# argmaxinc/WhisperKit

Hardware: NVIDIA H100
Metric: RTFx (audio-sec/s) whisper-large-v3 greedy (higher is better)
Workload: dtype bf16

## Files before the change

### whisperkit_b200/csrc/decoder_ops.cu

```cuda
#include <curand_kernel.h>
#include <math.h>

#include <stdlib.h>

#include "common.cuh"
#include <algorithm>
#include "kernels.h"

namespace wk {

static constexpr int kMaxCtx = 224;

__device__ __forceinline__ float block_sum(float v, float* scratch) {
    v = warp_sum(v);
    const int warp = threadIdx.x >> 5, lane = threadIdx.x & 31, nw = (blockDim.x + 31) >> 5;
    __syncthreads();
    if (lane == 0) scratch[warp] = v;
    __syncthreads();
    float r = (lane < nw) ? scratch[lane] : 0.f;
    r = warp_sum(r);
    return r;
}
__device__ __forceinline__ float block_max(float v, float* scratch) {
    v = warp_max(v);
    const int warp = threadIdx.x >> 5, lane = threadIdx.x & 31, nw = (blockDim.x + 31) >> 5;
    __syncthreads();
    if (lane == 0) scratch[warp] = v;
    __syncthreads();
    float r = (lane < nw) ? scratch[lane] : -INFINITY;
    r = warp_max(r);
    return r;
}

__global__ void decode_slots_init_kernel(DecodeState st, RowParams* __restrict__ rp_dev, const int32_t* __restrict__ slot_ids,
                                         const int32_t* __restrict__ prompts, const RowParams* __restrict__ rp_new, BeamState bs) {
    const int i = blockIdx.x, b = slot_ids[i];
    const RowParams R = rp_new[i];
    const int n_prompt = R.prompt_len;
    for (int t = threadIdx.x; t < kMaxCtx; t += blockDim.x) {
        st.tokens[b * kMaxCtx + t] = t < n_prompt ? prompts[i * kMaxCtx + t] : 0;
        st.logprobs[b * kMaxCtx + t] = 0.f;
        if (bs.beam > 1) bs.anc[b * kMaxCtx + t] = b;
    }
    if (threadIdx.x == 0) {
        rp_dev[b] = R;
        st.n_tokens[b] = n_prompt;
        st.next_token[b] = n_prompt > 0 ? prompts[i * kMaxCtx + n_prompt - 1] : 0;
        st.done[b] = 0;
        st.first_low[b] = 0;
        st.steps[b] = 0;
        st.input_ids[b] = 0;
        st.error[b] = 0;
        st.lang_token[b] = -1;
        st.lang_logprob[b] = 0.f;
        st.lang_state[b] = R.detect == 2 ? kLangLead : 0;
        st.no_speech[b] = __int_as_float(0x7fc00000);
        if (bs.beam > 1) {
            bs.sum_lp[b] = 0.f;
            if (b % bs.group == 0) bs.n_fin[b / bs.group] = 0;
        }
    }
}

wk_status decode_slots_init(DecodeState st, RowParams* rp_dev, const int32_t* slot_ids, const int32_t* prompts, const RowParams* rp_new,
                            int n, cudaStream_t stream, BeamState beam) {
    if (n < 1) return WK_OK;
    decode_slots_init_kernel<<<n, 64, 0, stream>>>(st, rp_dev, slot_ids, prompts, rp_new, beam);
    count_launch();
    cudaError_t e = cudaGetLastError();
    if (e != cudaSuccess) { set_error("decode_slots_init launch: %s", cudaGetErrorString(e)); return WK_ERR_CUDA; }
    return WK_OK;
}

template <typename T>
__global__ void __launch_bounds__(256)
decoder_embed_ln_kernel(const T* __restrict__ emb, const float* __restrict__ pos_emb, const float* __restrict__ gamma,
                        const float* __restrict__ beta, DecodeState st, int vocab, int ts_begin, float* __restrict__ x,
                        T* __restrict__ xn, int d, const int32_t* __restrict__ explicit_pos) {
    __shared__ float scratch[32];
    const int b = blockIdx.x, tid = threadIdx.x;
    pdl_launch_dependents();
    pdl_wait();
    int tok, pos;
    if (explicit_pos) {
        tok = st.input_ids[b];
        pos = explicit_pos[b];
    } else {
        if (st.done[b]) return;
        const int step = st.steps[b];
        const int prompt_len = st.rp[b].prompt_len;
        pos = step;
        tok = st.next_token[b];
        bool overwrite = false;
        const int lang_state = st.lang_state[b];
        if (lang_state == kLangLead) {
            tok = st.rp[b].lead_token;
        } else if (step < prompt_len) {
            const int cur = st.tokens[b * kMaxCtx + step];
            const bool is_ts = cur >= ts_begin, pred_ts = tok >= ts_begin;
            if (!(step == prompt_len - 1 && is_ts && pred_ts)) tok = cur;
            else overwrite = true;
        }
        __syncthreads();
        if (tid == 0) {
            if (overwrite) st.tokens[b * kMaxCtx + step] = tok;
            st.input_ids[b] = tok;
            if (lang_state == kLangLeadRan) st.lang_state[b] = 0;
        }
    }
    tok = min(max(tok, 0), vocab - 1);
    float v[8];
    float s = 0.f;
#pragma unroll
    for (int k = 0; k < 8; ++k) {
        const int i = tid + k * 256;
        v[k] = 0.f;
        if (i < d) {
            v[k] = T16<T>::to_f(emb[(long long)tok * d + i]) + pos_emb[(long long)pos * d + i];
            x[(long long)b * d + i] = v[k];
            s += v[k];
        }
    }
    const float mean = block_sum(s, scratch) / d;
    float q = 0.f;
#pragma unroll
    for (int k = 0; k < 8; ++k) {
        const int i = tid + k * 256;
        if (i < d) { const float a = v[k] - mean; q += a * a; }
    }
    const float rstd = rsqrtf(block_sum(q, scratch) / d + 1e-5f);
#pragma unroll
    for (int k = 0; k < 8; ++k) {
        const int i = tid + k * 256;
        if (i < d) xn[(long long)b * d + i] = T16<T>::from_f((v[k] - mean) * rstd * gamma[i] + beta[i]);
    }
}

wk_status decoder_embed_ln(const void* emb16, const float* pos, const float* gamma, const float* beta, DecodeState st, int vocab,
                           int ts_begin, float* x, void* xn, int B, int d, int dtype, const int32_t* explicit_pos, cudaStream_t stream) {
    if (d > 2048) { set_error("decoder_embed_ln: d_model %d > 2048", d); return WK_ERR_INVALID_ARGUMENT; }
    if (dtype == WK_DTYPE_F16)
        launch_k(decoder_embed_ln_kernel<__half>, dim3(B), dim3(256), 0, stream, 1, (const __half*)emb16, pos, gamma, beta, st, vocab, ts_begin, x, (__half*)xn, d, explicit_pos);
    else
        launch_k(decoder_embed_ln_kernel<__nv_bfloat16>, dim3(B), dim3(256), 0, stream, 1, (const __nv_bfloat16*)emb16, pos, gamma, beta, st, vocab, ts_begin, x, (__nv_bfloat16*)xn, d, explicit_pos);
    count_launch();
    cudaError_t e = cudaGetLastError();
    if (e != cudaSuccess) { set_error("decoder_embed_ln launch: %s", cudaGetErrorString(e)); return WK_ERR_CUDA; }
    return WK_OK;
}

static constexpr int kReduceThreads = 320;
static constexpr int kMaxSplits = 20;

template <typename T>
__global__ void __launch_bounds__(kReduceThreads)
decoder_reduce_resid_ln_kernel(const float* __restrict__ partial, int splits, int Bp, const float* __restrict__ bias,
                               const float* __restrict__ gamma, const float* __restrict__ beta, float* __restrict__ x,
                               T* __restrict__ xn, int d) {
    __shared__ float scratch[32];
    const int b = blockIdx.x, tid = threadIdx.x;
    const int d4 = d >> 2;
    pdl_launch_dependents();
    pdl_wait();
    float4 v[2];
    float s = 0.f;
#pragma unroll
    for (int k = 0; k < 2; ++k) {
        const int i4 = tid + k * kReduceThreads;
        v[k] = make_float4(0.f, 0.f, 0.f, 0.f);
        if (i4 < d4) {
            float4 p[kMaxSplits];
#pragma unroll
            for (int sp = 0; sp < kMaxSplits; ++sp)
                if (sp < splits) p[sp] = __ldcg(reinterpret_cast<const float4*>(partial + ((long long)sp * Bp + b) * d) + i4);
            float4 a = reinterpret_cast<const float4*>(x + (long long)b * d)[i4];
            if (bias) {
                const float4 bb = __ldg(reinterpret_cast<const float4*>(bias) + i4);
                a.x += bb.x; a.y += bb.y; a.z += bb.z; a.w += bb.w;
            }
#pragma unroll
            for (int sp = 0; sp < kMaxSplits; ++sp)
                if (sp < splits) { a.x += p[sp].x; a.y += p[sp].y; a.z += p[sp].z; a.w += p[sp].w; }
            v[k] = a;
            reinterpret_cast<float4*>(x + (long long)b * d)[i4] = a;
            s += a.x + a.y + a.z + a.w;
        }
    }
    const float mean = block_sum(s, scratch) / d;
    float q = 0.f;
#pragma unroll
    for (int k = 0; k < 2; ++k) {
        const int i4 = tid + k * kReduceThreads;
        if (i4 < d4) {
            const float a0 = v[k].x - mean, a1 = v[k].y - mean, a2 = v[k].z - mean, a3 = v[k].w - mean;
            q += a0 * a0 + a1 * a1 + a2 * a2 + a3 * a3;
        }
    }
    const float rstd = rsqrtf(block_sum(q, scratch) / d + 1e-5f);
#pragma unroll
    for (int k = 0; k < 2; ++k) {
        const int i4 = tid + k * kReduceThreads;
        if (i4 < d4) {
            const float4 g = __ldg(reinterpret_cast<const float4*>(gamma) + i4), bb = __ldg(reinterpret_cast<const float4*>(beta) + i4);
            uint2 pk;
            pk.x = T16<T>::pack2((v[k].x - mean) * rstd * g.x + bb.x, (v[k].y - mean) * rstd * g.y + bb.y);
            pk.y = T16<T>::pack2((v[k].z - mean) * rstd * g.z + bb.z, (v[k].w - mean) * rstd * g.w + bb.w);
            reinterpret_cast<uint2*>(xn + (long long)b * d)[i4] = pk;
        }
    }
}

wk_status decoder_reduce_resid_ln(const float* partial, int splits, int Bp, const float* bias, const float* gamma,
                                  const float* beta, float* x, void* xn, int B, int d, int dtype, cudaStream_t stream) {
    if (splits > kMaxSplits || d > 8 * kReduceThreads || (d & 3)) {
        set_error("decoder_reduce_resid_ln: unsupported splits %d / d %d", splits, d);
        return WK_ERR_INVALID_ARGUMENT;
    }
    if (dtype == WK_DTYPE_F16)
        launch_k(decoder_reduce_resid_ln_kernel<__half>, dim3(B), dim3(kReduceThreads), 0, stream, 32, partial, splits, Bp, bias, gamma, beta, x, (__half*)xn, d);
    else
        launch_k(decoder_reduce_resid_ln_kernel<__nv_bfloat16>, dim3(B), dim3(kReduceThreads), 0, stream, 32, partial, splits, Bp, bias, gamma, beta, x, (__nv_bfloat16*)xn, d);
    count_launch();
    cudaError_t e = cudaGetLastError();
    if (e != cudaSuccess) { set_error("decoder_reduce_resid_ln launch: %s", cudaGetErrorString(e)); return WK_ERR_CUDA; }
    return WK_OK;
}

template <typename T>
__global__ void __launch_bounds__(256)
decoder_reduce_bias_gelu_kernel(const float* __restrict__ partial, int splits, int Bp, const float* __restrict__ bias,
                                T* __restrict__ out, int B, int n) {
    pdl_launch_dependents();
    pdl_wait();
    const long long idx = ((long long)blockIdx.x * blockDim.x + threadIdx.x) * 4;
    if (idx >= (long long)B * n) return;
    const int b = (int)(idx / n), i = (int)(idx - (long long)b * n);
    float4 a = *reinterpret_cast<const float4*>(bias + i);
    float4 p[8];
#pragma unroll
    for (int sp = 0; sp < 8; ++sp)
        if (sp < splits) p[sp] = __ldcg(reinterpret_cast<const float4*>(partial + ((long long)sp * Bp + b) * n + i));
#pragma unroll
    for (int sp = 0; sp < 8; ++sp)
        if (sp < splits) { a.x += p[sp].x; a.y += p[sp].y; a.z += p[sp].z; a.w += p[sp].w; }
    for (int sp = 8; sp < splits; ++sp) {
        const float4 pp = __ldcg(reinterpret_cast<const float4*>(partial + ((long long)sp * Bp + b) * n + i));
        a.x += pp.x; a.y += pp.y; a.z += pp.z; a.w += pp.w;
    }
    uint2 pk;
    pk.x = T16<T>::pack2(gelu_erf(a.x), gelu_erf(a.y));
    pk.y = T16<T>::pack2(gelu_erf(a.z), gelu_erf(a.w));
    *reinterpret_cast<uint2*>(out + (long long)b * n + i) = pk;
}

wk_status decoder_reduce_bias_gelu(const float* partial, int splits, int Bp, const float* bias, void* out, int B, int n,
                                   int dtype, cudaStream_t stream) {
    const long long threads = (long long)B * n / 4;
    const unsigned grid = (unsigned)((threads + 255) / 256);
    if (dtype == WK_DTYPE_F16)
        launch_k(decoder_reduce_bias_gelu_kernel<__half>, dim3(grid), dim3(256), 0, stream, 32, partial, splits, Bp, bias, (__half*)out, B, n);
    else
        launch_k(decoder_reduce_bias_gelu_kernel<__nv_bfloat16>, dim3(grid), dim3(256), 0, stream, 32, partial, splits, Bp, bias, (__nv_bfloat16*)out, B, n);
    count_launch();
    cudaError_t e = cudaGetLastError();
    if (e != cudaSuccess) { set_error("decoder_reduce_bias_gelu launch: %s", cudaGetErrorString(e)); return WK_ERR_CUDA; }
    return WK_OK;
}

template <typename T, bool kAnc>
__global__ void __launch_bounds__(128)
decoder_self_attention_kernel(const float* __restrict__ partial, int splits, int Bp, const float* __restrict__ bq,
                              const float* __restrict__ bv, T* __restrict__ kcache, T* __restrict__ vcache,
                              const int32_t* __restrict__ pos_ptr, const int32_t* __restrict__ done,
                              T* __restrict__ out, int B, int H, int max_len, const int32_t* __restrict__ anc) {
    __shared__ float sq[64], skc[64], svc[64];
    __shared__ float sp[kMaxCtx];
    __shared__ float red[4][64];
    __shared__ float sstat[8];
    const int tid = threadIdx.x, warp = tid >> 5, lane = tid & 31;
    const int bh = blockIdx.x, b = bh / H, h = bh % H;
    pdl_launch_dependents();
    pdl_wait();
    if (done != nullptr && done[b]) return;
    const int dm = H * 64;
    const int pos = pos_ptr[b];
    const int32_t* arow = kAnc ? anc + (long long)b * max_len : nullptr;
    const long long own = (long long)bh * max_len;
    auto row_of = [&](int t) -> long long { return kAnc ? ((long long)arow[t] * H + h) * max_len + t : own + t; };
    if (warp == 0) {
        const int e = 2 * lane;
        float2 q = make_float2(bq[h * 64 + e], bq[h * 64 + e + 1]);
        float2 k = make_float2(0.f, 0.f);
        float2 v = make_float2(bv[h * 64 + e], bv[h * 64 + e + 1]);
        for (int s = 0; s < splits; ++s) {
            const float* pr = partial + ((long long)s * Bp + b) * (3LL * dm) + h * 64 + e;
            const float2 pq = *reinterpret_cast<const float2*>(pr);
            const float2 pk = *reinterpret_cast<const float2*>(pr + dm);
            const float2 pv = *reinterpret_cast<const float2*>(pr + 2 * dm);
            q.x += pq.x; q.y += pq.y; k.x += pk.x; k.y += pk.y; v.x += pv.x; v.y += pv.y;
        }
        const uint32_t k16 = T16<T>::pack2(k.x, k.y), v16 = T16<T>::pack2(v.x, v.y);
        *reinterpret_cast<uint32_t*>(kcache + (own + pos) * 64 + e) = k16;
        *reinterpret_cast<uint32_t*>(vcache + (own + pos) * 64 + e) = v16;
        const float2 kr = T16<T>::unpack2(k16), vr = T16<T>::unpack2(v16);
        sq[e] = q.x; sq[e + 1] = q.y;
        skc[e] = kr.x; skc[e + 1] = kr.y;
        svc[e] = vr.x; svc[e + 1] = vr.y;
        const float self = warp_sum(q.x * kr.x + q.y * kr.y);
        if (lane == 0) sp[pos] = self * 0.125f;
    }
    __syncthreads();
    const int sub = lane & 7, rsel = lane >> 3;
    float qv[8];
#pragma unroll
    for (int j = 0; j < 8; ++j) qv[j] = sq[sub * 8 + j];
    const T* kb = kcache + sub * 8;
#pragma unroll 4
    for (int t0 = warp * 4; t0 < pos; t0 += 16) {
        const int t = t0 + rsel;
        float acc = 0.f;
        if (t < pos) {
            const uint4 u = *reinterpret_cast<const uint4*>(kb + row_of(t) * 64);
            const float2 a0 = T16<T>::unpack2(u.x), a1 = T16<T>::unpack2(u.y), a2 = T16<T>::unpack2(u.z), a3 = T16<T>::unpack2(u.w);
            acc = qv[0] * a0.x + qv[1] * a0.y + qv[2] * a1.x + qv[3] * a1.y + qv[4] * a2.x + qv[5] * a2.y + qv[6] * a3.x + qv[7] * a3.y;
        }
        acc += __shfl_xor_sync(0xffffffffu, acc, 1);
        acc += __shfl_xor_sync(0xffffffffu, acc, 2);
        acc += __shfl_xor_sync(0xffffffffu, acc, 4);
        if (sub == 0 && t < pos) sp[t] = acc * 0.125f;
    }
    __syncthreads();
    float mx = -INFINITY;
    for (int t = tid; t <= pos; t += 128) mx = fmaxf(mx, sp[t]);
    mx = warp_max(mx);
    if (lane == 0) sstat[warp] = mx;
    __syncthreads();
    mx = fmaxf(fmaxf(sstat[0], sstat[1]), fmaxf(sstat[2], sstat[3]));
    float sm = 0.f;
    for (int t = tid; t <= pos; t += 128) {
        const float pr = __expf(sp[t] - mx);
        sp[t] = pr;
        sm += pr;
    }
    sm = warp_sum(sm);
    if (lane == 0) sstat[4 + warp] = sm;
    __syncthreads();
    const float inv = 1.f / (sstat[4] + sstat[5] + sstat[6] + sstat[7]);
    float o8[8];
#pragma unroll
    for (int j = 0; j < 8; ++j) o8[j] = 0.f;
    const T* vb = vcache + sub * 8;
#pragma unroll 4
    for (int t0 = warp * 4; t0 < pos; t0 += 16) {
        const int t = t0 + rsel;
        if (t < pos) {
            const float pr = sp[t];
            const uint4 u = *reinterpret_cast<const uint4*>(vb + row_of(t) * 64);
            const float2 a0 = T16<T>::unpack2(u.x), a1 = T16<T>::unpack2(u.y), a2 = T16<T>::unpack2(u.z), a3 = T16<T>::unpack2(u.w);
            o8[0] += pr * a0.x; o8[1] += pr * a0.y; o8[2] += pr * a1.x; o8[3] += pr * a1.y;
            o8[4] += pr * a2.x; o8[5] += pr * a2.y; o8[6] += pr * a3.x; o8[7] += pr * a3.y;
        }
    }
#pragma unroll
    for (int j = 0; j < 8; ++j) {
        o8[j] += __shfl_xor_sync(0xffffffffu, o8[j], 8);
        o8[j] += __shfl_xor_sync(0xffffffffu, o8[j], 16);
    }
    if (rsel == 0) {
#pragma unroll
        for (int j = 0; j < 8; ++j) red[warp][sub * 8 + j] = o8[j];
    }
    __syncthreads();
    if (tid < 64) {
        const float o = red[0][tid] + red[1][tid] + red[2][tid] + red[3][tid] + sp[pos] * svc[tid];
        out[(long long)b * dm + h * 64 + tid] = T16<T>::from_f(o * inv);
    }
}

wk_status decoder_self_attention(const float* partial, int splits, int Bp, const float* bq, const float* bv, void* kcache,
                                 void* vcache, const int32_t* pos, const int32_t* done, void* out, int B, int H,
                                 int max_len, int dtype, cudaStream_t stream, const int32_t* anc) {
    if (max_len > kMaxCtx) { set_error("decoder_self_attention: max_len %d > %d", max_len, kMaxCtx); return WK_ERR_INVALID_ARGUMENT; }
    const unsigned grid = (unsigned)(B * H);
    if (dtype == WK_DTYPE_F16) {
        if (anc) launch_k(decoder_self_attention_kernel<__half, true>, dim3(grid), dim3(128), 0, stream, 2, partial, splits, Bp, bq, bv, (__half*)kcache, (__half*)vcache, pos, done, (__half*)out, B, H, max_len, anc);
        else launch_k(decoder_self_attention_kernel<__half, false>, dim3(grid), dim3(128), 0, stream, 2, partial, splits, Bp, bq, bv, (__half*)kcache, (__half*)vcache, pos, done, (__half*)out, B, H, max_len, anc);
    } else {
        if (anc) launch_k(decoder_self_attention_kernel<__nv_bfloat16, true>, dim3(grid), dim3(128), 0, stream, 2, partial, splits, Bp, bq, bv, (__nv_bfloat16*)kcache, (__nv_bfloat16*)vcache, pos, done, (__nv_bfloat16*)out, B, H, max_len, anc);
        else launch_k(decoder_self_attention_kernel<__nv_bfloat16, false>, dim3(grid), dim3(128), 0, stream, 2, partial, splits, Bp, bq, bv, (__nv_bfloat16*)kcache, (__nv_bfloat16*)vcache, pos, done, (__nv_bfloat16*)out, B, H, max_len, anc);
    }
    count_launch();
    cudaError_t e = cudaGetLastError();
    if (e != cudaSuccess) { set_error("decoder_self_attention launch: %s", cudaGetErrorString(e)); return WK_ERR_CUDA; }
    return WK_OK;
}

template <bool FP8> struct CrossCfg {
    static constexpr int kRowBytes = FP8 ? 64 : 128;
    static constexpr int kRows = FP8 ? 250 : 125;
    static constexpr int kStageBytes = kRows * kRowBytes;
    static constexpr int kStages = 2;
    static constexpr int kLanesPerRow = kRowBytes / 16;
    static constexpr int kRowsPerWarp = 32 / kLanesPerRow;
    static constexpr int kDims = 64 / kLanesPerRow;
};
static constexpr int kCrossRows = CrossCfg<false>::kRows;
static constexpr int kCrossThreads = 160;

__device__ __forceinline__ void fp8x16_to_f32(const uint4 u, float (&x)[16]) {
    const uint32_t w[4] = {u.x, u.y, u.z, u.w};
#pragma unroll
    for (int k = 0; k < 4; ++k) {
        uint32_t lo, hi;
        fp8x4_to_half2(w[k], lo, hi);
        const float2 a = T16<__half>::unpack2(lo), b = T16<__half>::unpack2(hi);
        x[4 * k] = a.x; x[4 * k + 1] = a.y; x[4 * k + 2] = b.x; x[4 * k + 3] = b.y;
    }
}
template <typename T, bool FP8>
__device__ __forceinline__ float cross_row_dot(const uint8_t* piece, const float (&qv)[CrossCfg<FP8>::kDims]) {
    const uint4 u = *reinterpret_cast<const uint4*>(piece);
    if constexpr (FP8) {
        float x[16];
        fp8x16_to_f32(u, x);
        float acc = 0.f;
#pragma unroll
        for (int j = 0; j < 16; ++j) acc = fmaf(qv[j], x[j], acc);
        return acc;
    } else {
        const float2 a0 = T16<T>::unpack2(u.x), a1 = T16<T>::unpack2(u.y), a2 = T16<T>::unpack2(u.z), a3 = T16<T>::unpack2(u.w);
        return qv[0] * a0.x + qv[1] * a0.y + qv[2] * a1.x + qv[3] * a1.y + qv[4] * a2.x + qv[5] * a2.y + qv[6] * a3.x + qv[7] * a3.y;
    }
}
template <typename T, bool FP8>
__device__ __forceinline__ void cross_row_axpy(const uint8_t* piece, float p, float (&acc)[CrossCfg<FP8>::kDims]) {
    const uint4 u = *reinterpret_cast<const uint4*>(piece);
    if constexpr (FP8) {
        float x[16];
        fp8x16_to_f32(u, x);
#pragma unroll
        for (int j = 0; j < 16; ++j) acc[j] = fmaf(p, x[j], acc[j]);
    } else {
        const float2 a0 = T16<T>::unpack2(u.x), a1 = T16<T>::unpack2(u.y), a2 = T16<T>::unpack2(u.z), a3 = T16<T>::unpack2(u.w);
        acc[0] += p * a0.x; acc[1] += p * a0.y; acc[2] += p * a1.x; acc[3] += p * a1.y;
        acc[4] += p * a2.x; acc[5] += p * a2.y; acc[6] += p * a3.x; acc[7] += p * a3.y;
    }
}

template <typename T, bool FP8>
__global__ void __launch_bounds__(kCrossThreads)
decoder_cross_attention_kernel(const float* __restrict__ partial, int splits, int Bp, const float* __restrict__ bq,
                               const uint8_t* __restrict__ kcross, const uint8_t* __restrict__ vcross, const float* __restrict__ kscale,
                               const float* __restrict__ vscale, T* __restrict__ out, int B, int H, int Tlen, const int32_t* __restrict__ done,
                               float* __restrict__ align_scratch, uint32_t align_mask, int kv_div) {
    using C = CrossCfg<FP8>;
    extern __shared__ __align__(128) uint8_t smem[];
    const int Tp = (Tlen + 3) & ~3;
    uint8_t* ring = smem;
    float* scores = reinterpret_cast<float*>(smem + C::kStages * C::kStageBytes);
    float* ksc = scores + Tp;
    float* vsc = ksc + Tp;
    float* sq = FP8 ? vsc + Tp : scores + Tp;
    float* red = sq + 64;
    uint64_t* full_bar = reinterpret_cast<uint64_t*>(red + 4 * 64 + 32);
    uint64_t* empty_bar = full_bar + C::kStages;
    uint64_t* scale_bar = empty_bar + C::kStages;

    const int tid = threadIdx.x, warp = tid >> 5, lane = tid & 31;
    const int beam_j = blockIdx.x % kv_div, wh = blockIdx.x / kv_div;
    const int win = wh / H, h = wh % H, b = win * kv_div + beam_j;
    const int kvh = win * H + h;
    const int dm = H * 64;
    const int chunks = Tlen / C::kRows;
    pdl_launch_dependents();
    const int ended = done != nullptr ? done[b] : 0;
    if (tid == 0) {
        for (int i = 0; i < C::kStages; ++i) { mbar_init(&full_bar[i], 1); mbar_init(&empty_bar[i], 4); }
        if constexpr (FP8) mbar_init(scale_bar, 1);
        fence_barrier_init();
    }
    __syncthreads();
    if (ended) { pdl_wait(); return; }

    if (warp == 4) {
        if (lane == 0) {
            if constexpr (FP8) {
                mbar_expect_tx(scale_bar, 2u * Tlen * 4);
                bulk_load_1d(ksc, kscale + (long long)kvh * Tlen, Tlen * 4, scale_bar);
                bulk_load_1d(vsc, vscale + (long long)kvh * Tlen, Tlen * 4, scale_bar);
            }
            const uint8_t* kb = kcross + (long long)kvh * Tlen * C::kRowBytes;
            const uint8_t* vb = vcross + (long long)kvh * Tlen * C::kRowBytes;
            for (int c = 0; c < 2 * chunks; ++c) {
                const int stage = c % C::kStages;
                const uint32_t ph = (c / C::kStages) & 1;
                mbar_wait(&empty_bar[stage], ph ^ 1);
                mbar_expect_tx(&full_bar[stage], C::kStageBytes);
                const uint8_t* src = c < chunks ? kb + (long long)c * C::kStageBytes : vb + (long long)(c - chunks) * C::kStageBytes;
                bulk_load_1d(ring + stage * C::kStageBytes, src, C::kStageBytes, &full_bar[stage]);
            }
        }
        return;
    }
    pdl_wait();
    if (tid < 64) {
        float q = bq[h * 64 + tid];
        for (int s = 0; s < splits; ++s) q += partial[((long long)s * Bp + b) * dm + h * 64 + tid];
        sq[tid] = q * 0.125f;
    }
    asm volatile("bar.sync 1, 128;" ::: "memory");
    const int sub = lane % C::kLanesPerRow;
    const int rsel = lane / C::kLanesPerRow;
    float qv[C::kDims];
#pragma unroll
    for (int j = 0; j < C::kDims; ++j) qv[j] = sq[sub * C::kDims + j];
    if constexpr (FP8) mbar_wait(scale_bar, 0);

    for (int c = 0; c < chunks; ++c) {
        const int stage = c % C::kStages;
        const uint32_t ph = (c / C::kStages) & 1;
        mbar_wait(&full_bar[stage], ph);
        const uint8_t* tile = ring + stage * C::kStageBytes;
#pragma unroll
        for (int i = 0; i < 8; ++i) {
            const int r = warp * C::kRowsPerWarp + rsel + 4 * C::kRowsPerWarp * i;
            float acc = 0.f;
            if (r < C::kRows) acc = cross_row_dot<T, FP8>(tile + r * C::kRowBytes + sub * 16, qv);
#pragma unroll
            for (int o = 1; o < C::kLanesPerRow; o <<= 1) acc += __shfl_xor_sync(0xffffffffu, acc, o);
            if (sub == 0 && r < C::kRows) scores[c * C::kRows + r] = FP8 ? acc * ksc[c * C::kRows + r] : acc;
        }
        __syncwarp();
        if (lane == 0) mbar_arrive(&empty_bar[stage]);
    }
    asm volatile("bar.sync 1, 128;" ::: "memory");
    float mx = -INFINITY;
    for (int t = tid; t < Tlen; t += 128) mx = fmaxf(mx, scores[t]);
    mx = warp_max(mx);
    if (lane == 0) red[warp] = mx;
    asm volatile("bar.sync 1, 128;" ::: "memory");
    mx = fmaxf(fmaxf(red[0], red[1]), fmaxf(red[2], red[3]));
    float sm = 0.f;
    for (int t = tid; t < Tlen; t += 128) {
        const float p = __expf(scores[t] - mx);
        scores[t] = p;
        sm += p;
    }
    sm = warp_sum(sm);
    asm volatile("bar.sync 1, 128;" ::: "memory");
    if (lane == 0) red[warp] = sm;
    asm volatile("bar.sync 1, 128;" ::: "memory");
    const float inv = 1.f / (red[0] + red[1] + red[2] + red[3]);
    if (align_scratch != nullptr && ((align_mask >> h) & 1u)) {
        const int slot = __popc(align_mask & ((1u << h) - 1u));
        float* dst = align_scratch + ((long long)slot * B + b) * Tlen;
        for (int t = tid; t < Tlen; t += 128) dst[t] = scores[t] * inv;
    }

    float acc[C::kDims];
#pragma unroll
    for (int j = 0; j < C::kDims; ++j) acc[j] = 0.f;
    for (int c = chunks; c < 2 * chunks; ++c) {
        const int stage = c % C::kStages;
        const uint32_t ph = (c / C::kStages) & 1;
        mbar_wait(&full_bar[stage], ph);
        const uint8_t* tile = ring + stage * C::kStageBytes;
#pragma unroll
        for (int i = 0; i < 8; ++i) {
            const int r = warp * C::kRowsPerWarp + rsel + 4 * C::kRowsPerWarp * i;
            if (r < C::kRows) {
                const int t = (c - chunks) * C::kRows + r;
                const float p = FP8 ? scores[t] * vsc[t] : scores[t];
                cross_row_axpy<T, FP8>(tile + r * C::kRowBytes + sub * 16, p, acc);
            }
        }
        __syncwarp();
        if (lane == 0) mbar_arrive(&empty_bar[stage]);
    }
#pragma unroll
    for (int j = 0; j < C::kDims; ++j) {
#pragma unroll
        for (int o = C::kLanesPerRow; o < 32; o <<= 1) acc[j] += __shfl_xor_sync(0xffffffffu, acc[j], o);
    }
    asm volatile("bar.sync 1, 128;" ::: "memory");
    if (rsel == 0) {
#pragma unroll
        for (int j = 0; j < C::kDims; ++j) red[warp * 64 + sub * C::kDims + j] = acc[j];
    }
    asm volatile("bar.sync 1, 128;" ::: "memory");
    if (tid < 64) {
        const float o = (red[tid] + red[64 + tid] + red[128 + tid] + red[192 + tid]) * inv;
        out[(long long)b * dm + h * 64 + tid] = T16<T>::from_f(o);
    }
}

template <bool FP8> static size_t cross_smem_bytes(int T) {
    using C = CrossCfg<FP8>;
    return (size_t)C::kStages * C::kStageBytes + (size_t)((T + 3) & ~3) * 4 * (FP8 ? 3 : 1) + 64 * 4 + (4 * 64 + 32) * 4 +
           (2 * C::kStages + (FP8 ? 1 : 0)) * 8 + 64;
}

template <typename T, bool FP8>
static wk_status launch_cross(const float* partial, int splits, int Bp, const float* bq, const void* kcross, const void* vcross, const float* kscale,
                              const float* vscale, void* out, int B, int H, int Tlen, cudaStream_t stream, const int32_t* done, float* align_scratch,
                              uint32_t align_mask, int kv_div) {
    static bool attr_set = false;
    if (!attr_set) {
        cudaError_t e = cudaFuncSetAttribute(decoder_cross_attention_kernel<T, FP8>, cudaFuncAttributeMaxDynamicSharedMemorySize, 100 * 1024);
        if (e != cudaSuccess) { set_error("cudaFuncSetAttribute(cross): %s", cudaGetErrorString(e)); return WK_ERR_CUDA; }
        attr_set = true;
    }
    launch_k(decoder_cross_attention_kernel<T, FP8>, dim3(B * H), dim3(kCrossThreads), cross_smem_bytes<FP8>(Tlen), stream, 4, partial, splits, Bp, bq,
             (const uint8_t*)kcross, (const uint8_t*)vcross, kscale, vscale, (T*)out, B, H, Tlen, done, align_scratch, align_mask, kv_div);
    return WK_OK;
}


__global__ void decoder_align_mean_kernel(const float* __restrict__ scratch, int n_slots, const int32_t* __restrict__ steps,
                                          const int32_t* __restrict__ done, const int32_t* __restrict__ lang_state, __half* __restrict__ out,
                                          int B, int Tlen, int max_rows) {
    const int b = blockIdx.y, t = blockIdx.x * blockDim.x + threadIdx.x;
    const int row = steps[b];
    if (t >= Tlen || row >= max_rows || done[b] || (lang_state != nullptr && lang_state[b] == kLangLeadRan)) return;
    float a = 0.f;
    for (int s = 0; s < n_slots; ++s) a += scratch[((long long)s * B + b) * Tlen + t];
    out[((long long)b * max_rows + row) * Tlen + t] = __float2half(a / (float)n_slots);
}

wk_status decoder_align_mean(const float* scratch, int n_slots, const int32_t* steps, const int32_t* done, const int32_t* lang_state,
                             void* out_f16, int B, int T, int max_rows, cudaStream_t stream) {
    launch_k(decoder_align_mean_kernel, dim3((T + 255) / 256, B), dim3(256), 0, stream, 0, scratch, n_slots, steps, done, lang_state, (__half*)out_f16, B, T, max_rows);
    count_launch();
    cudaError_t e = cudaGetLastError();
    if (e != cudaSuccess) { set_error("decoder_align_mean launch: %s", cudaGetErrorString(e)); return WK_ERR_CUDA; }
    return WK_OK;
}

wk_status decoder_cross_attention(const float* partial, int splits, int Bp, const float* bq, const void* kcross,
                                  const void* vcross, void* out, int B, int H, int T, int dtype, cudaStream_t stream,
                                  const int32_t* done, float* align_scratch, uint32_t align_mask, int kv_div, const float* kscale,
                                  const float* vscale) {
    const bool fp8 = kscale != nullptr;
    if (kv_div < 1 || B % kv_div != 0) { set_error("decoder_cross_attention: %d rows do not split into groups of %d", B, kv_div); return WK_ERR_INVALID_ARGUMENT; }
    if (!fp8 && T % kCrossRows != 0) { set_error("decoder_cross_attention: n_audio_ctx %d not a multiple of %d", T, kCrossRows); return WK_ERR_INVALID_ARGUMENT; }
    if (kv_div > 1 && kv_div <= 8 && align_scratch == nullptr)
        return decoder_cross_attention_mq(partial, splits, Bp, bq, kcross, vcross, out, B, H, T, dtype, stream, done, kv_div, kscale, vscale);
    if (fp8 && (T % CrossCfg<true>::kRows != 0 || T % 4 != 0)) { set_error("decoder_cross_attention (fp8): n_audio_ctx %d not a multiple of 500", T); return WK_ERR_INVALID_ARGUMENT; }
    const bool f16 = dtype == WK_DTYPE_F16;
    wk_status st = fp8 ? (f16 ? launch_cross<__half, true>(partial, splits, Bp, bq, kcross, vcross, kscale, vscale, out, B, H, T, stream, done, align_scratch, align_mask, kv_div)
                              : launch_cross<__nv_bfloat16, true>(partial, splits, Bp, bq, kcross, vcross, kscale, vscale, out, B, H, T, stream, done, align_scratch, align_mask, kv_div))
                       : (f16 ? launch_cross<__half, false>(partial, splits, Bp, bq, kcross, vcross, kscale, vscale, out, B, H, T, stream, done, align_scratch, align_mask, kv_div)
                              : launch_cross<__nv_bfloat16, false>(partial, splits, Bp, bq, kcross, vcross, kscale, vscale, out, B, H, T, stream, done, align_scratch, align_mask, kv_div));
    if (st != WK_OK) return st;
    count_launch();
    cudaError_t e = cudaGetLastError();
    if (e != cudaSuccess) { set_error("decoder_cross_attention launch: %s", cudaGetErrorString(e)); return WK_ERR_CUDA; }
    return WK_OK;
}

static constexpr int kSamplerThreads = 1024;

struct ArgMax { float v; int i; };
__device__ __forceinline__ ArgMax argmax_better(ArgMax a, ArgMax b) {
    if (b.v > a.v || (b.v == a.v && b.i < a.i)) return b;
// ... 454 lines not shown
```

### whisperkit_b200/csrc/engine.cu

```cuda
#include <math.h>
#include <stdarg.h>
#include <stdio.h>
#include <stdlib.h>
#include <string.h>
#include <dirent.h>

#include <algorithm>
#include <atomic>
#include <map>
#include <memory>
#include <string>
#include <vector>

#include "common.cuh"
#include "engine.h"

namespace wk {

static thread_local char g_err[1024] = "";
void set_error(const char* fmt, ...) {
    va_list ap;
    va_start(ap, fmt);
    vsnprintf(g_err, sizeof(g_err), fmt, ap);
    va_end(ap);
}
const char* last_error_cstr() { return g_err; }
static std::atomic<long long> g_launches{0};
static std::atomic<int64_t> g_live_bytes[2] = {{0}, {0}};
static std::atomic<int> g_pdl{-1};
int pdl_mode() {
    int v = g_pdl.load(std::memory_order_relaxed);
    if (v < 0) {
        v = 53;
        if (const char* e = getenv("WKB200_PDL_MASK")) v = (int)strtol(e, nullptr, 0) & 63;
        g_pdl.store(v, std::memory_order_relaxed);
    }
    return v;
}
bool pdl_enabled() { return pdl_mode() > 0; }
void pdl_disable() { g_pdl.store(0, std::memory_order_relaxed); }
void count_launch(int n) { g_launches.fetch_add(n, std::memory_order_relaxed); }
long long launch_counter_load() { return g_launches.load(); }
void launch_counter_sub(long long n) { g_launches.fetch_sub(n); }

wk_status Buffers::alloc(void** p, size_t bytes, bool pinned, bool zero) {
    cudaError_t e = pinned ? cudaHostAlloc(p, bytes, cudaHostAllocDefault) : cudaMalloc(p, bytes);
    if (e != cudaSuccess) {
        cudaGetLastError();
        *p = nullptr;
        if (pinned) set_error("pinned staging of %zu bytes failed: %s", bytes, cudaGetErrorString(e));
        else set_error("cudaMalloc(%zu bytes) failed: %s", bytes, cudaGetErrorString(e));
        return WK_ERR_CUDA;
    }
    live_.push_back({*p, bytes, pinned});
    g_live_bytes[pinned].fetch_add((int64_t)bytes);
    if (zero) {
        if (pinned) memset(*p, 0, bytes);
        else if ((e = cudaMemset(*p, 0, bytes)) != cudaSuccess) { set_error("cudaMemset failed: %s", cudaGetErrorString(e)); return WK_ERR_CUDA; }
    }
    return WK_OK;
}

static void free_buffer(void* p, size_t bytes, bool pinned) {
    if (pinned) cudaFreeHost(p);
    else cudaFree(p);
    g_live_bytes[pinned].fetch_sub((int64_t)bytes);
}

wk_status Buffers::regrow(void** p, size_t bytes, bool pinned, cudaStream_t drain, bool* moved) {
    if (moved) *moved = false;
    auto it = std::find_if(live_.begin(), live_.end(), [&](const Buf& b) { return *p && b.p == *p; });
    if ((it == live_.end() ? 0 : it->bytes) >= bytes) return WK_OK;
    if (moved) *moved = true;
    if (it != live_.end()) {
        if (drain) WK_CUDA_CHECK(cudaStreamSynchronize(drain));
        free_buffer(it->p, it->bytes, it->pinned);
        live_.erase(it);
    }
    return alloc(p, bytes, pinned, false);
}

void Buffers::release_all() {
    for (const Buf& b : live_) free_buffer(b.p, b.bytes, b.pinned);
    live_.clear();
}

int choose_splits(int tiles, int total_kb, int num_sms) {
    int best = 1;
    for (int s = 1; s <= total_kb && s <= 20; ++s) {
        if (total_kb % s) continue;
        if (tiles * s <= num_sms) best = s;
    }
    return best;
}

size_t esize(int dtype) { return dtype == WK_DTYPE_F32 || dtype == WK_DTYPE_I32 ? 4 : 2; }

static wk_status alloc_ln(Buffers& b, LayerNormW& ln, int d) {
    WK_CHECK(b.dmalloc(&ln.g, d));
    WK_CHECK(b.dmalloc(&ln.b, d));
    return WK_OK;
}

static wk_status model_alloc(wk_model* m) {
    const wk_model_config& c = m->cfg;
    const int d = c.d_model, L = c.enc_layers, Ld = c.dec_layers;
    const size_t T = c.n_audio_ctx;
    Buffers& b = m->mem;
    WK_CHECK(b.alloc16(&m->conv1_w, (size_t)d * 3 * 128));
    WK_CHECK(b.dmalloc(&m->conv1_b, d));
    WK_CHECK(b.alloc16(&m->conv2_w, (size_t)d * 3 * d));
    WK_CHECK(b.dmalloc(&m->conv2_b, d));
    WK_CHECK(b.dmalloc(&m->enc_pos, T * d));
    m->enc.resize(L);
    for (auto& l : m->enc) {
        WK_CHECK(alloc_ln(b, l.ln1, d)); WK_CHECK(alloc_ln(b, l.ln2, d));
        WK_CHECK(b.alloc16(&l.wqkv, (size_t)3 * d * d)); WK_CHECK(b.dmalloc(&l.bqkv, 3 * d));
        WK_CHECK(b.alloc16(&l.wo, (size_t)d * d)); WK_CHECK(b.dmalloc(&l.bo, d));
        WK_CHECK(b.alloc16(&l.w1, (size_t)4 * d * d)); WK_CHECK(b.dmalloc(&l.b1, 4 * d));
        WK_CHECK(b.alloc16(&l.w2, (size_t)4 * d * d)); WK_CHECK(b.dmalloc(&l.b2, d));
    }
    WK_CHECK(alloc_ln(b, m->enc_ln, d));
    WK_CHECK(b.alloc16(&m->emb, (size_t)round_up(c.vocab, 128) * d));
    WK_CHECK(b.dmalloc(&m->dec_pos, (size_t)c.n_text_ctx * d));
    m->dec.resize(Ld);
    for (auto& l : m->dec) {
        WK_CHECK(alloc_ln(b, l.ln1, d)); WK_CHECK(alloc_ln(b, l.lnx, d)); WK_CHECK(alloc_ln(b, l.ln3, d));
        WK_CHECK(b.alloc16(&l.wqkv, (size_t)3 * d * d)); WK_CHECK(b.dmalloc(&l.bq, d)); WK_CHECK(b.dmalloc(&l.bv, d));
        WK_CHECK(b.alloc16(&l.wo, (size_t)d * d)); WK_CHECK(b.dmalloc(&l.bo, d));
        WK_CHECK(b.alloc16(&l.wcq, (size_t)d * d)); WK_CHECK(b.dmalloc(&l.bcq, d));
        WK_CHECK(b.alloc16(&l.wco, (size_t)d * d)); WK_CHECK(b.dmalloc(&l.bco, d));
        WK_CHECK(b.alloc16(&l.w1, (size_t)4 * d * d)); WK_CHECK(b.dmalloc(&l.b1, 4 * d));
        WK_CHECK(b.alloc16(&l.w2, (size_t)4 * d * d)); WK_CHECK(b.dmalloc(&l.b2, d));
    }
    WK_CHECK(alloc_ln(b, m->dec_ln, d));
    WK_CHECK(b.alloc16(&m->wckv, (size_t)2 * Ld * d * d));
    WK_CHECK(b.dmalloc(&m->bckv, (size_t)2 * Ld * d));
    return WK_OK;
}

wk_status enc_ws_ensure(wk_model* m, EncWorkspace* ws, int max_batch) {
    if (ws->max_batch >= max_batch) return WK_OK;
    *ws = EncWorkspace();
    const wk_model_config& c = m->cfg;
    const int d = c.d_model, Bm = max_batch;
    const size_t T = c.n_audio_ctx;
    Buffers& b = ws->mem;
    WK_CHECK(b.dmalloc(&ws->pcm_dev, (size_t)Bm * kWindowSamples, false));
    WK_CHECK(b.dmalloc(&ws->nvalid_dev, Bm));
    WK_CHECK(b.dmalloc(&ws->gmax, Bm));
    WK_CHECK(b.alloc16(&ws->mel, (size_t)Bm * kMelRows * kMelCols));
    WK_CHECK(b.alloc16(&ws->h1, (size_t)Bm * kMelRows * d));
    const size_t M = (size_t)Bm * T;
    WK_CHECK(b.dmalloc(&ws->x, M * d, false));
    WK_CHECK(b.alloc16(&ws->xn, M * d));
    WK_CHECK(b.alloc16(&ws->qkv, M * 3 * d));
    WK_CHECK(b.alloc16(&ws->attn, M * d));
    WK_CHECK(b.alloc16(&ws->ffn, M * 4 * d));
    WK_CHECK(b.alloc16(&ws->enc_out, M * d));
    ws->max_batch = Bm;
    return WK_OK;
}

__global__ void conv_w_rearrange_kernel(const float* __restrict__ src, __half* __restrict__ dst, int co, int ci, int ci_pad) {
    const long long idx = (long long)blockIdx.x * blockDim.x + threadIdx.x;
    const long long n = (long long)co * 3 * ci_pad;
    if (idx >= n) return;
    const int c = (int)(idx % ci_pad);
    const int tap = (int)((idx / ci_pad) % 3);
    const int o = (int)(idx / (3LL * ci_pad));
    dst[idx] = c < ci ? __float2half_rn(src[((long long)o * ci + c) * 3 + tap]) : __float2half_rn(0.f);
}

struct Dest { void* p; int dtype; size_t numel; int special; };

static bool resolve_name(wk_model* m, const std::string& name, Dest* out) {
    const int d = m->cfg.d_model, dt = m->cfg.dtype;
    auto W = [&](void* p, size_t rows_off, size_t n) { *out = {(char*)p + rows_off * (size_t)d * 2, dt, n, 0}; return true; };
    auto F = [&](float* p, size_t n) { *out = {p, WK_DTYPE_F32, n, 0}; return true; };
    int i = -1;
    char rest[128];
    if (name == "model.encoder.conv1.weight") { *out = {m->conv1_w, WK_DTYPE_F16, (size_t)d * m->cfg.n_mels * 3, 1}; return true; }
    if (name == "model.encoder.conv1.bias") return F(m->conv1_b, d);
    if (name == "model.encoder.conv2.weight") { *out = {m->conv2_w, WK_DTYPE_F16, (size_t)d * d * 3, 2}; return true; }
    if (name == "model.encoder.conv2.bias") return F(m->conv2_b, d);
    if (name == "model.encoder.embed_positions.weight") return F(m->enc_pos, (size_t)m->cfg.n_audio_ctx * d);
    if (name == "model.encoder.layer_norm.weight") return F(m->enc_ln.g, d);
    if (name == "model.encoder.layer_norm.bias") return F(m->enc_ln.b, d);
    if (name == "model.decoder.embed_tokens.weight" || name == "proj_out.weight") { *out = {m->emb, dt, (size_t)m->cfg.vocab * d, 0}; return true; }
    if (name == "model.decoder.embed_positions.weight") return F(m->dec_pos, (size_t)m->cfg.n_text_ctx * d);
    if (name == "model.decoder.layer_norm.weight") return F(m->dec_ln.g, d);
    if (name == "model.decoder.layer_norm.bias") return F(m->dec_ln.b, d);
    if (sscanf(name.c_str(), "model.encoder.layers.%d.%127s", &i, rest) == 2 && i >= 0 && i < (int)m->enc.size()) {
        EncLayer& l = m->enc[i];
        const std::string r = rest;
        const size_t dd = (size_t)d * d;
        if (r == "self_attn.q_proj.weight") return W(l.wqkv, 0, dd);
        if (r == "self_attn.k_proj.weight") return W(l.wqkv, d, dd);
        if (r == "self_attn.v_proj.weight") return W(l.wqkv, 2 * (size_t)d, dd);
        if (r == "self_attn.q_proj.bias") return F(l.bqkv, d);
        if (r == "self_attn.k_proj.bias") return F(l.bqkv + d, d);
        if (r == "self_attn.v_proj.bias") return F(l.bqkv + 2 * d, d);
        if (r == "self_attn.out_proj.weight") return W(l.wo, 0, dd);
        if (r == "self_attn.out_proj.bias") return F(l.bo, d);
        if (r == "self_attn_layer_norm.weight") return F(l.ln1.g, d);
        if (r == "self_attn_layer_norm.bias") return F(l.ln1.b, d);
        if (r == "final_layer_norm.weight") return F(l.ln2.g, d);
        if (r == "final_layer_norm.bias") return F(l.ln2.b, d);
        if (r == "fc1.weight") return W(l.w1, 0, 4 * dd);
        if (r == "fc1.bias") return F(l.b1, 4 * (size_t)d);
        if (r == "fc2.weight") return W(l.w2, 0, 4 * dd);
        if (r == "fc2.bias") return F(l.b2, d);
        return false;
    }
    if (sscanf(name.c_str(), "model.decoder.layers.%d.%127s", &i, rest) == 2 && i >= 0 && i < (int)m->dec.size()) {
        DecLayer& l = m->dec[i];
        const std::string r = rest;
        const size_t dd = (size_t)d * d;
        if (r == "self_attn.q_proj.weight") return W(l.wqkv, 0, dd);
        if (r == "self_attn.k_proj.weight") return W(l.wqkv, d, dd);
        if (r == "self_attn.v_proj.weight") return W(l.wqkv, 2 * (size_t)d, dd);
        if (r == "self_attn.q_proj.bias") return F(l.bq, d);
        if (r == "self_attn.v_proj.bias") return F(l.bv, d);
        if (r == "self_attn.out_proj.weight") return W(l.wo, 0, dd);
        if (r == "self_attn.out_proj.bias") return F(l.bo, d);
        if (r == "self_attn_layer_norm.weight") return F(l.ln1.g, d);
        if (r == "self_attn_layer_norm.bias") return F(l.ln1.b, d);
        if (r == "encoder_attn.q_proj.weight") return W(l.wcq, 0, dd);
        if (r == "encoder_attn.q_proj.bias") return F(l.bcq, d);
        if (r == "encoder_attn.k_proj.weight") return W(m->wckv, (size_t)(2 * i) * d, dd);
        if (r == "encoder_attn.v_proj.weight") return W(m->wckv, (size_t)(2 * i + 1) * d, dd);
        if (r == "encoder_attn.v_proj.bias") return F(m->bckv + (size_t)(2 * i + 1) * d, d);
        if (r == "encoder_attn.out_proj.weight") return W(l.wco, 0, dd);
        if (r == "encoder_attn.out_proj.bias") return F(l.bco, d);
        if (r == "encoder_attn_layer_norm.weight") return F(l.lnx.g, d);
        if (r == "encoder_attn_layer_norm.bias") return F(l.lnx.b, d);
        if (r == "final_layer_norm.weight") return F(l.ln3.g, d);
        if (r == "final_layer_norm.bias") return F(l.ln3.b, d);
        if (r == "fc1.weight") return W(l.w1, 0, 4 * dd);
        if (r == "fc1.bias") return F(l.b1, 4 * (size_t)d);
        if (r == "fc2.weight") return W(l.w2, 0, 4 * dd);
        if (r == "fc2.bias") return F(l.b2, d);
        return false;
    }
    return false;
}

GemmDesc plain_gemm(const void* a, int64_t M, int K, const void* w, int N, int dtype, int mode, void* out, int64_t ld_out,
                    const float* bias, int gelu) {
    GemmDesc g;
    memset(&g, 0, sizeof(g));
    g.a = a; g.a_rows = M; g.a_cols = K; g.a_ld = K; g.a_batches = 1;
    g.b = w; g.b_rows = N; g.b_ld = K; g.in_dtype = dtype;
    g.m_rows_per_batch = (int)M; g.n = N; g.k = K; g.taps = 1;
    g.bn = N >= 256 ? 256 : round_up(N, 16);
    g.splits = 1; g.mode = mode; g.gelu = gelu; g.out = out; g.ld_out = ld_out; g.out_rows_per_batch = M; g.bias = bias;
    return g;
}

wk_status mel_run(wk_model* m, EncWorkspace* ws, const float* pcm, int64_t n, int64_t stride, const int32_t* samples_per_window,
                  void* mel_out, cudaStream_t stream) {
    if (n < 1 || n > ws->max_batch) { set_error("log-mel: %lld windows outside [1, %d]", (long long)n, ws->max_batch); return WK_ERR_AUDIO_PROCESSING_FAILED; }
    if (stride < kWindowSamples && !samples_per_window) { set_error("log-mel: stride %lld < 480000 requires samples_per_window", (long long)stride); return WK_ERR_AUDIO_PROCESSING_FAILED; }
    cudaPointerAttributes at;
    const bool on_device = cudaPointerGetAttributes(&at, pcm) == cudaSuccess && at.type == cudaMemoryTypeDevice;
    cudaGetLastError();
    const float* src = pcm;
    int64_t src_stride = stride;
    if (!on_device || stride < kWindowSamples) {
        if (stride < kWindowSamples) WK_CUDA_CHECK(cudaMemsetAsync(ws->pcm_dev, 0, (size_t)n * kWindowSamples * 4, stream));
        WK_CUDA_CHECK(cudaMemcpy2DAsync(ws->pcm_dev, kWindowSamples * 4, pcm, stride * 4, std::min<int64_t>(stride, kWindowSamples) * 4, n,
                                        cudaMemcpyDefault, stream));
        src = ws->pcm_dev;
        src_stride = kWindowSamples;
    }
    const int32_t* nv = nullptr;
    if (samples_per_window) {
        for (int64_t i = 0; i < n; ++i)
            if (samples_per_window[i] < 0 || samples_per_window[i] > kWindowSamples) { set_error("log-mel: samples_per_window[%lld] out of range", (long long)i); return WK_ERR_AUDIO_PROCESSING_FAILED; }
        WK_CUDA_CHECK(cudaMemcpyAsync(ws->nvalid_dev, samples_per_window, n * 4, cudaMemcpyHostToDevice, stream));
        nv = ws->nvalid_dev;
    }
    return mel_forward(&m->mel_tables, src, n, src_stride, nv, mel_out, ws->gmax, stream);
}

static GemmDesc fp8_gemm(const uint8_t* a, const float* a_scale, int64_t ld, int64_t M, int K, const uint8_t* w, const float* w_scale, int N,
                         int dtype, int mode, void* out, float* out_scale, const float* bias, int gelu) {
    GemmDesc g = plain_gemm(a, M, K, w, N, dtype, mode, out, N, bias, gelu);
    g.a_ld = K; g.b_ld = K;
    g.a_scale = a_scale; g.a_scale_ld = ld; g.w_scale = w_scale; g.out_scale = out_scale;
    return g;
}

static wk_status encode_layers_fp8(wk_model* m, EncWorkspace* ws, int B, void* enc_out, cudaStream_t s) {
    const wk_model_config& c = m->cfg;
    const int d = c.d_model, T = c.n_audio_ctx, dt = c.dtype;
    const int64_t M = (int64_t)B * T;
    const int64_t ld = round_up(ws->max_batch * T, 128);
    if (!ws->xn_scale) {
        WK_CHECK(ws->mem.dmalloc(&ws->xn_scale, (size_t)(d / kFp8Block) * ld));
        WK_CHECK(ws->mem.dmalloc(&ws->ffn_scale, (size_t)(4 * d / kFp8Block) * ld));
    }
    uint8_t* xn8 = static_cast<uint8_t*>(ws->xn);
    uint8_t* ffn8 = static_cast<uint8_t*>(ws->ffn);
    for (int li = 0; li < c.enc_layers; ++li) {
        EncLayer& l = m->enc[li];
        WK_CHECK(layernorm_f32_to_fp8(ws->x, l.ln1.g, l.ln1.b, xn8, ws->xn_scale, ld, M, d, s));
        WK_CHECK(gemm_wgmma_fp8(fp8_gemm(xn8, ws->xn_scale, ld, M, d, l.wqkv8, l.sqkv, 3 * d, dt, GEMM_OUT_T16, ws->qkv, nullptr, l.bqkv, 0),
                                m->num_sms, s));
        WK_CHECK(encoder_attention(ws->qkv, ws->attn, B, T, c.n_heads, dt, s));
        WK_CHECK(gemm_wgmma(plain_gemm(ws->attn, M, d, l.wo, d, dt, GEMM_OUT_F32_ADD, ws->x, d, l.bo, 0), m->num_sms, s));
        WK_CHECK(layernorm_f32_to_fp8(ws->x, l.ln2.g, l.ln2.b, xn8, ws->xn_scale, ld, M, d, s));
        WK_CHECK(gemm_wgmma_fp8(fp8_gemm(xn8, ws->xn_scale, ld, M, d, l.w18, l.s1, 4 * d, dt, GEMM_OUT_FP8_BLOCKS, ffn8, ws->ffn_scale, l.b1, 1),
                                m->num_sms, s));
        WK_CHECK(gemm_wgmma_fp8(fp8_gemm(ffn8, ws->ffn_scale, ld, M, 4 * d, l.w28, l.s2, d, dt, GEMM_OUT_F32_ADD, ws->x, nullptr, l.b2, 0),
                                m->num_sms, s));
    }
    WK_CHECK(layernorm_f32_to_16(ws->x, m->enc_ln.g, m->enc_ln.b, enc_out, M, d, dt, s));
    return WK_OK;
}

static wk_status quantize_enc_layer(wk_model* m, int li) {
    const int d = m->cfg.d_model, dt = m->cfg.dtype;
    EncLayer& l = m->enc[li];
    WK_CHECK(quantize_weight_rows_fp8(l.wqkv, dt, l.wqkv8, l.sqkv, 3 * d, d, m->stream));
    WK_CHECK(quantize_weight_rows_fp8(l.w1, dt, l.w18, l.s1, 4 * d, d, m->stream));
    WK_CHECK(quantize_weight_rows_fp8(l.w2, dt, l.w28, l.s2, d, 4 * d, m->stream));
    return WK_OK;
}

static wk_status quantize_enc_weights(wk_model* m) {
    for (size_t li = 0; li < m->enc.size(); ++li) WK_CHECK(quantize_enc_layer(m, (int)li));
    WK_CUDA_CHECK(cudaStreamSynchronize(m->stream));
    return WK_OK;
}

// ... 943 lines not shown
```

Measured before the change: 957.7.

## Stage decoder self-attention KV reads through a cp.async ring before PDL wait

The decoder self-attention kernel now loads past K and V cache rows into a 4-stage shared-memory ring with cp.async, 32 rows per stage, and consumes them from shared memory. The first stages are issued before the grid-dependency wait, so cache reads overlap the previous kernel's tail. The default PDL mask also changes from 53 to 55, enabling PDL on one more kernel group. This adds about 16KB of shared memory per block and extra block barriers per stage, which may reduce occupancy. Prefetching before the wait relies on the cached rows not being written by the upstream kernel.

```diff
diff --git a/whisperkit_b200/csrc/decoder_ops.cu b/whisperkit_b200/csrc/decoder_ops.cu
--- a/whisperkit_b200/csrc/decoder_ops.cu
+++ b/whisperkit_b200/csrc/decoder_ops.cu
@@ -267,12 +267,16 @@
     return WK_OK;
 }
 
+static constexpr int kSelfRows = 32;
+static constexpr int kSelfStages = 4;
+
 template <typename T, bool kAnc>
 __global__ void __launch_bounds__(128)
 decoder_self_attention_kernel(const float* __restrict__ partial, int splits, int Bp, const float* __restrict__ bq,
                               const float* __restrict__ bv, T* __restrict__ kcache, T* __restrict__ vcache,
                               const int32_t* __restrict__ pos_ptr, const int32_t* __restrict__ done,
                               T* __restrict__ out, int B, int H, int max_len, const int32_t* __restrict__ anc) {
+    __shared__ __align__(16) uint4 ring[kSelfStages][kSelfRows * 8];
     __shared__ float sq[64], skc[64], svc[64];
     __shared__ float sp[kMaxCtx];
     __shared__ float red[4][64];
@@ -280,13 +284,36 @@
     const int tid = threadIdx.x, warp = tid >> 5, lane = tid & 31;
     const int bh = blockIdx.x, b = bh / H, h = bh % H;
     pdl_launch_dependents();
-    pdl_wait();
-    if (done != nullptr && done[b]) return;
+    if (done != nullptr && done[b]) { pdl_wait(); return; }
     const int dm = H * 64;
     const int pos = pos_ptr[b];
     const int32_t* arow = kAnc ? anc + (long long)b * max_len : nullptr;
     const long long own = (long long)bh * max_len;
     auto row_of = [&](int t) -> long long { return kAnc ? ((long long)arow[t] * H + h) * max_len + t : own + t; };
+    const int nk = (pos + kSelfRows - 1) / kSelfRows;
+    auto issue = [&](int g) {
+        if (g < 2 * nk) {
+            const T* src = g < nk ? kcache : vcache;
+            const int t0 = (g < nk ? g : g - nk) * kSelfRows;
+            uint4* stage = ring[g % kSelfStages];
+#pragma unroll
+            for (int i = 0; i < kSelfRows * 8 / 128; ++i) {
+                const int pc = tid + 128 * i, r = pc >> 3, s = pc & 7;
+                if (t0 + r < pos) cp_async16(stage + pc, src + row_of(t0 + r) * 64 + s * 8, true);
+            }
+        }
+        cp_async_commit();
+    };
+    auto consume = [&](int g, int t0, auto&& f) {
+        cp_async_wait<kSelfStages - 1>();
+        __syncthreads();
+        f(ring[g % kSelfStages], t0);
+        __syncthreads();
+        issue(g + kSelfStages);
+    };
+#pragma unroll
+    for (int g = 0; g < kSelfStages; ++g) issue(g);
+    pdl_wait();
     if (warp == 0) {
         const int e = 2 * lane;
         float2 q = make_float2(bq[h * 64 + e], bq[h * 64 + e + 1]);
@@ -314,20 +341,23 @@
     float qv[8];
 #pragma unroll
     for (int j = 0; j < 8; ++j) qv[j] = sq[sub * 8 + j];
-    const T* kb = kcache + sub * 8;
-#pragma unroll 4
-    for (int t0 = warp * 4; t0 < pos; t0 += 16) {
-        const int t = t0 + rsel;
-        float acc = 0.f;
-        if (t < pos) {
-            const uint4 u = *reinterpret_cast<const uint4*>(kb + row_of(t) * 64);
-            const float2 a0 = T16<T>::unpack2(u.x), a1 = T16<T>::unpack2(u.y), a2 = T16<T>::unpack2(u.z), a3 = T16<T>::unpack2(u.w);
-            acc = qv[0] * a0.x + qv[1] * a0.y + qv[2] * a1.x + qv[3] * a1.y + qv[4] * a2.x + qv[5] * a2.y + qv[6] * a3.x + qv[7] * a3.y;
-        }
-        acc += __shfl_xor_sync(0xffffffffu, acc, 1);
-        acc += __shfl_xor_sync(0xffffffffu, acc, 2);
-        acc += __shfl_xor_sync(0xffffffffu, acc, 4);
-        if (sub == 0 && t < pos) sp[t] = acc * 0.125f;
+    for (int g = 0; g < nk; ++g) {
+        consume(g, g * kSelfRows, [&](const uint4* stage, int c0) {
+#pragma unroll
+            for (int i = 0; i < kSelfRows / 16; ++i) {
+                const int r = 16 * i + 4 * warp + rsel, t = c0 + r;
+                float acc = 0.f;
+                if (t < pos) {
+                    const uint4 u = stage[r * 8 + sub];
+                    const float2 a0 = T16<T>::unpack2(u.x), a1 = T16<T>::unpack2(u.y), a2 = T16<T>::unpack2(u.z), a3 = T16<T>::unpack2(u.w);
+                    acc = qv[0] * a0.x + qv[1] * a0.y + qv[2] * a1.x + qv[3] * a1.y + qv[4] * a2.x + qv[5] * a2.y + qv[6] * a3.x + qv[7] * a3.y;
+                }
+                acc += __shfl_xor_sync(0xffffffffu, acc, 1);
+                acc += __shfl_xor_sync(0xffffffffu, acc, 2);
+                acc += __shfl_xor_sync(0xffffffffu, acc, 4);
+                if (sub == 0 && t < pos) sp[t] = acc * 0.125f;
+            }
+        });
     }
     __syncthreads();
     float mx = -INFINITY;
@@ -349,17 +379,20 @@
     float o8[8];
 #pragma unroll
     for (int j = 0; j < 8; ++j) o8[j] = 0.f;
-    const T* vb = vcache + sub * 8;
-#pragma unroll 4
-    for (int t0 = warp * 4; t0 < pos; t0 += 16) {
-        const int t = t0 + rsel;
-        if (t < pos) {
-            const float pr = sp[t];
-            const uint4 u = *reinterpret_cast<const uint4*>(vb + row_of(t) * 64);
-            const float2 a0 = T16<T>::unpack2(u.x), a1 = T16<T>::unpack2(u.y), a2 = T16<T>::unpack2(u.z), a3 = T16<T>::unpack2(u.w);
-            o8[0] += pr * a0.x; o8[1] += pr * a0.y; o8[2] += pr * a1.x; o8[3] += pr * a1.y;
-            o8[4] += pr * a2.x; o8[5] += pr * a2.y; o8[6] += pr * a3.x; o8[7] += pr * a3.y;
-        }
+    for (int g = nk; g < 2 * nk; ++g) {
+        consume(g, (g - nk) * kSelfRows, [&](const uint4* stage, int c0) {
+#pragma unroll
+            for (int i = 0; i < kSelfRows / 16; ++i) {
+                const int r = 16 * i + 4 * warp + rsel, t = c0 + r;
+                if (t < pos) {
+                    const float pr = sp[t];
+                    const uint4 u = stage[r * 8 + sub];
+                    const float2 a0 = T16<T>::unpack2(u.x), a1 = T16<T>::unpack2(u.y), a2 = T16<T>::unpack2(u.z), a3 = T16<T>::unpack2(u.w);
+                    o8[0] += pr * a0.x; o8[1] += pr * a0.y; o8[2] += pr * a1.x; o8[3] += pr * a1.y;
+                    o8[4] += pr * a2.x; o8[5] += pr * a2.y; o8[6] += pr * a3.x; o8[7] += pr * a3.y;
+                }
+            }
+        });
     }
 #pragma unroll
     for (int j = 0; j < 8; ++j) {
diff --git a/whisperkit_b200/csrc/engine.cu b/whisperkit_b200/csrc/engine.cu
--- a/whisperkit_b200/csrc/engine.cu
+++ b/whisperkit_b200/csrc/engine.cu
@@ -31,7 +31,7 @@
 int pdl_mode() {
     int v = g_pdl.load(std::memory_order_relaxed);
     if (v < 0) {
-        v = 53;
+        v = 55;
         if (const char* e = getenv("WKB200_PDL_MASK")) v = (int)strtol(e, nullptr, 0) & 63;
         g_pdl.store(v, std::memory_order_relaxed);
     }
```

Result: no change. 967.2, median of 6 (+1.0%).
